# yhwu/rsicnv

Hardware: AMD Instinct MI355X
Metric: bases/sec through RSI pipeline (bin+GC+NB+segment) (higher is better)
Workload: dtype int32

## Files before the change

rsicnv_amd/csrc/kernels.h:

```cpp
#pragma once
#include <hip/hip_runtime.h>
#include <stdint.h>
#include <mutex>
#include "device_util.h"
#include "bam_walk_core.h"

namespace rsik {

inline void note_launch() {
  const hipError_t e = hipGetLastError();
  if (e != hipSuccess && tl_launch_error == hipSuccess) tl_launch_error = e;
}
inline void drain_stale_errors() { (void)hipGetLastError(); tl_launch_error = hipSuccess; }
inline hipError_t take_launch_error() { const hipError_t e = tl_launch_error; tl_launch_error = hipSuccess; return e; }
#define RSI_LAUNCH(...) do { hipLaunchKernelGGL(__VA_ARGS__); rsik::note_launch(); } while (0)

constexpr int kGcLevels = 202;
constexpr int kHistValues = 65536;
constexpr int kResClasses = 32;
constexpr int kTileBases = 4096;

void launch_fasta_classify(const uint8_t* fasta, int64_t n, uint64_t* gcbits, uint64_t* nbits, int64_t nwords,
                           const FillList& fill, hipStream_t stream);
void launch_fill(const FillList& fill, hipStream_t stream);
// ... 149 lines not shown
                    double dup_raw, double RDmedian, void* ws, uint32_t* rawmin_bits, const GridChain& c, GridMedian* g,
                    const GridExport* ex, const FillList* fill, hipStream_t stream);
void launch_nb_apply(const int64_t* binsum, int64_t nb, int64_t K, const void* ws, float* T, const FillList* fill, hipStream_t stream);

struct ScanParams {
  int64_t nb;
  int32_t Lmax;
  int16_t pad;
  int16_t kcap;
  double tmedian;
  double lim_del;
  double lim_dup;
};
constexpr int kMaxScanL = 10400;
constexpr int kScanLdsL = 3800;
constexpr int kScanPad = 8;
constexpr int kThrInline = 232;
struct ScanThr { double del[kThrInline]; double dup[kThrInline]; };
void launch_rsi_scan(const float* T, const int32_t* medint, const ScanParams& sp, const double* thr_del,
                     const double* thr_dup, const ScanThr* inl, uint32_t* first_del, uint32_t* first_dup, uint32_t* counters,
                     uint32_t* tiles, void* tile_ws , hipStream_t stream);
size_t scan_tile_workspace_bytes(int Lmax);
constexpr int kMaxLevels = 10416;
inline int scan_level_stride(int Lmax) { return (Lmax + 1 + kScanPad + 3) & ~3; }
constexpr int kScanRecEscapes = 0, kScanRecInexact = 1, kScanRecStop = 2 , kScanRecTiles = 8, kScanRecLevels = 16;
constexpr size_t kScanWorkBytes = 64 + 2 * (size_t)kMaxLevels * 4;
void launch_level_stop(const uint32_t* first_del, const uint32_t* first_dup, int64_t nb, int32_t Lmax, uint32_t* work, void* both,
                       unsigned int* counter, void* host_copy, size_t host_bytes, hipStream_t stream);
void launch_resolve_runs(const uint32_t* first_del, const uint32_t* first_dup, const uint32_t* levels, int64_t nb, int32_t* status,
                         int32_t* copy, uint64_t* runs, uint32_t* count, uint32_t cap, unsigned int* counter, void* host_copy,
                         uint32_t host_entries, hipStream_t stream);

struct BestSeg { double score; int32_t start; int32_t len; };
struct SegItem { int32_t run; int32_t len; int32_t Lbeg; int32_t Lend; };
constexpr int kRunsInline = 200, kItemsInline = 150;
constexpr int kBestLds = 6144;
struct RunsInline { int32_t se[2 * kRunsInline]; int32_t off[kRunsInline]; };
struct ItemsInline { SegItem it[kItemsInline]; int32_t off[kRunsInline]; };
void launch_run_prefix(const float* T, const int32_t* run_start, const int32_t* run_end, const RunsInline* inl, int nruns,
                       const int64_t* poff, double* scratch, const int32_t* status, int32_t* status_out, hipStream_t stream);
void launch_best_items(const void* items, const ItemsInline* inl, int nitems, const int64_t* poff, const double* scratch,
                       double tmedian, BestSeg* out, hipStream_t stream);
void launch_trim_runs(const float* T, int32_t* status, const int32_t* run_start, const int32_t* run_end, const RunsInline* inl,
                      int nruns, double delthr, double addthr, hipStream_t stream);

size_t level_sums_head_bytes(int Lmax_cap);
size_t level_sums_workspace_bytes(int64_t nb, int32_t clist_cap, int Lmax_cap);
void launch_level_sums(const float* T, const int32_t* status, int64_t nb, int Lmax, void* ws, int Lmax_cap, int32_t clist_cap, float* out,
                       unsigned int* counter, void* host_copy, hipStream_t stream);

constexpr int kMaxDevices = 16;
void report_attribute_failure(const char* kernel, const char* what);
#define RSI_ALLOW_FULL_LDS(kernel)                                                                                  \
  do {                                                                                                              \
    static std::once_flag once__[rsik::kMaxDevices];                                                                \
    int dev__ = 0;                                                                                                  \
    if (hipGetDevice(&dev__) != hipSuccess || dev__ < 0 || dev__ >= rsik::kMaxDevices) dev__ = 0;                   \
    std::call_once(once__[dev__], [dev__] {                                                                         \
      hipFuncAttributes a__;                                                                                        \
      int lds__ = 0;                                                                                                \
      if (hipFuncGetAttributes(&a__, reinterpret_cast<const void*>(kernel)) != hipSuccess) {                        \
        rsik::report_attribute_failure(#kernel, "hipFuncGetAttributes"); return;                                    \
      }                                                                                                             \
      if (hipDeviceGetAttribute(&lds__, hipDeviceAttributeMaxSharedMemoryPerBlock, dev__) != hipSuccess || lds__ <= 0) \
        lds__ = 160 * 1024;                                                                                         \
      if (hipFuncSetAttribute(reinterpret_cast<const void*>(kernel), hipFuncAttributeMaxDynamicSharedMemorySize,   \
                              lds__ - (int)a__.sharedSizeBytes) != hipSuccess)                                      \
        rsik::report_attribute_failure(#kernel, "hipFuncSetAttribute(MaxDynamicSharedMemorySize)");                 \
    });                                                                                                             \
  } while (0)

constexpr unsigned kCandHistBins = 16384;
struct EdgeJob {
  int32_t start, end, type, pad;
};
struct CandJob {
  int32_t start, end;
  int32_t kind;
  int32_t margin;
  int32_t capacity;
  int32_t top;
  int32_t nleft, nright;
  int32_t left_off, right_off;
  int32_t budget;
  int32_t cut;
  double right_cap;
  int64_t iscratch_off;
  int64_t lscratch_off;
};
struct CandOut {
  int32_t flags;
  int32_t nref, nbody, nwin, left_reach, right_reach, body_min, body_max;
  double body_q[3], body_s1, body_s2;
  double ref_q[3], ref_s1, ref_s2;
};
struct DepthRef { const void* p; int bytes; };
void launch_widen_u8(const uint8_t* src, int64_t n, int32_t* dst, hipStream_t stream);
void launch_patch_i32(int32_t* dst, const int32_t* pos, const int32_t* val, int64_t cnt, hipStream_t stream);
void launch_range_sums(DepthRef rdc, const void* ranges , int nranges, long long* sums, hipStream_t stream);
void launch_sharpen_edges(DepthRef rdc, int64_t ncompact, EdgeJob* jobs, int njobs, void* ws, int ws_jobs, hipStream_t stream);
size_t sharpen_workspace_bytes(int njobs);
size_t sharpen_workspace_zero_bytes(int njobs);
inline size_t cand_scratch_bytes(int top, int capacity, int budget, int value_bytes, bool split) {
  auto up16 = [](size_t x) { return (x + 15) & ~size_t(15); };
  const size_t vb = (size_t)value_bytes;
  return up16((size_t)(top + 1 > 0 ? top + 1 : 0) * vb) + up16((size_t)capacity * 4) +
         up16((size_t)(capacity < budget ? capacity : budget) * vb) + (split ? up16((size_t)capacity * vb) : 0);
}
constexpr int kCandChunks = 16;
struct CandMid {
  int32_t lcnt, lreach, lused, rcnt_max, rreach, rused;
  uint32_t done, body_flags;
  float flo[kCandChunks], fhi[kCandChunks];
  double m1[kCandChunks], m2[kCandChunks];
  int32_t body_min, body_max;
  double body_q[3], body_s1, body_s2;
};
void launch_candidate_test_split(DepthRef rdc, int64_t ncompact, const CandJob* jobs, int njobs, const void* chains,
                                 int32_t* iscratch, double RDmedian, CandMid* mid, uint32_t* ghist,
                                 CandOut* outs, int value_bytes, hipStream_t stream);
void launch_candidate_test(DepthRef rdc, int64_t ncompact, const CandJob* jobs, int njobs, const void* chains,
                           int32_t* iscratch, long long* lscratch, double RDmedian, CandOut* outs, int value_bytes, hipStream_t stream);

struct TextParseStats { unsigned long long lines, stored, beyond; unsigned int unsorted, pad; };
int text_parse_workgroups(long long nbytes);
void launch_parse_depth_text(const void* text, long long nbytes, long long size, int32_t* depth, long long* wg_first,
                             long long* wg_max, TextParseStats* stats, hipStream_t stream);

struct NameBound { long long line; int32_t name, len; };
void launch_text_name_bounds(const void* text, long long nbytes, NameBound* bounds, unsigned int* count, unsigned int cap,
                             hipStream_t stream, bool bedgraph = false);
struct GenomeSeg { long long start, n; int32_t* depth; int32_t slot, pad; };
struct GenomeSlotStats { unsigned long long lines, stored, beyond; unsigned int unsorted, pad; long long last_pos;  };
constexpr int kMaxGenomeSegs = 512;
constexpr int kMaxGenomeSamples = 64;
// ... 162 lines not shown
```

rsicnv_amd/csrc/kernels_bin.hip:

```cpp
#include <type_traits>
#include "kernels.h"
#include "device_util.h"

namespace rsik {

namespace {

constexpr int kThreads = 256;
constexpr int kMaxGrid = 256 * 2;

__device__ inline int lane_id() { return threadIdx.x & 63; }
inline int grid_for(int64_t items, int per_block) {
  int64_t g = (items + per_block - 1) / per_block;
  if (g < 1) g = 1;
  if (g > kMaxGrid) g = kMaxGrid;
  return (int)g;
}

__device__ inline uint32_t f32_key(float f) {
  const uint32_t b = __float_as_uint(f);
  return (b & 0x80000000u) ? ~b : (b | 0x80000000u);
}

__device__ __forceinline__ float nb_raw_value(double sum, double m2, double r) {
// ... 1176 lines not shown
                                                        const int32_t* __restrict__ run_end, int nruns, double delthr,
                                                        double addthr, RunsInline inl) {
  __shared__ int s_min[kThreads / 64];
  const int r = blockIdx.x;
  if (r >= nruns) return;
  const int s = run_start ? run_start[r] : inl.se[2 * r], e = run_start ? run_end[r] : inl.se[2 * r + 1];
  auto pred = [&](int i) { const int st = status[i]; const double t = (double)T[i]; return (t > delthr && st < 0) || (t < addthr && st > 0); };
  auto first_failure = [&](int origin, int dir, int limit) {
    int done = 0;
    while (done < limit) {
      const int i = done + (int)threadIdx.x;
      int f = (i < limit && pred(origin + dir * i)) ? 0x7fffffff : i;
      for (int d = 32; d >= 1; d >>= 1) { const int o = __shfl_xor(f, d); f = o < f ? o : f; }
      __syncthreads();
      if ((threadIdx.x & 63) == 0) s_min[threadIdx.x >> 6] = f;
      __syncthreads();
      f = s_min[0];
      for (int w = 1; w < kThreads / 64; ++w) f = s_min[w] < f ? s_min[w] : f;
      if (f != 0x7fffffff) return f < limit ? f : limit;
      done += kThreads;
    }
    return limit;
  };
  const int lim_left = s < e ? e - s : 1;
  const int zl = first_failure(s, +1, lim_left);
  const int L = s + zl;
  int zr = 0;
  if (s < e) zr = first_failure(e, -1, e - L > 1 ? e - L : 1);
  __syncthreads();
  for (int i = threadIdx.x; i < zl; i += kThreads) status[s + i] = 0;
  for (int i = threadIdx.x; i < zr; i += kThreads) status[e - i] = 0;
}

__global__ __launch_bounds__(kThreads) void k_run_prefix(const float* __restrict__ T, const int32_t* __restrict__ run_start,
                                                         const int32_t* __restrict__ run_end,
                                                         const int64_t* __restrict__ poff, double* __restrict__ scratch, RunsInline inl,
                                                         const int32_t* __restrict__ status, int32_t* __restrict__ status_out) {
  __shared__ double s_tot[kThreads];
  const int r = blockIdx.x;
  const int s = run_start ? run_start[r] : inl.se[2 * r];
  const int len = (run_start ? run_end[r] : inl.se[2 * r + 1]) - s + 1;
  const int64_t off = poff ? poff[r] : (int64_t)inl.off[r];
  double* P = scratch + off;
  if (status_out) for (int e = threadIdx.x; e < len; e += kThreads) status_out[off - r + e] = status[s + e];
  const int chunk = (len + kThreads - 1) / kThreads;
  const int c0 = threadIdx.x * chunk;
  double run = 0.0;
  for (int e = c0; e < c0 + chunk && e < len; ++e) run += (double)T[s + e];
  s_tot[threadIdx.x] = run;
  __syncthreads();
  if (threadIdx.x < 64) {
    double carry = 0.0;
    for (int k = 0; k < kThreads / 64; ++k) {
      const double mine = s_tot[k * 64 + threadIdx.x];
      const double incl = wave_incl_scan(mine);
      s_tot[k * 64 + threadIdx.x] = carry + incl - mine;
      carry += wave_lane63(incl);
    }
  }
  __syncthreads();
  run = s_tot[threadIdx.x];
  if (threadIdx.x == 0) P[0] = 0.0;
  for (int e = c0; e < c0 + chunk && e < len; ++e) { run += (double)T[s + e]; P[e + 1] = run; }
}

__device__ inline bool seg_better(double s, int L, int j, double bs, int bL, int bj) {
  if (s != bs) return s > bs;
  if (L != bL) return L < bL;
  return j < bj;
}

__global__ __launch_bounds__(kThreads) void k_best_subsegment(const SegItem* __restrict__ items,
                                                              const int64_t* __restrict__ poff,
                                                              const double* __restrict__ scratch, double tmedian,
                                                              BestSeg* __restrict__ out, ItemsInline inl) {
  __shared__ double s_s[kThreads];
  __shared__ int s_L[kThreads], s_j[kThreads];
  const SegItem it = items ? items[blockIdx.x] : inl.it[blockIdx.x];
  const double* P = scratch + (poff ? poff[it.run] : (int64_t)inl.off[it.run]);
  double bs = -1.0; int bL = 0x7fffffff, bj = 0x7fffffff;
  __shared__ double s_P[kBestLds];
  const bool staged = it.len + 1 <= kBestLds;
  if (staged) for (int e = threadIdx.x; e <= it.len; e += kThreads) s_P[e] = P[e];
  __syncthreads();
  const double* Q = staged ? s_P : P;
  for (int L0 = it.Lbeg; L0 < it.Lend; L0 += 4) {
    double dL[4], sq[4];
#pragma unroll
    for (int u = 0; u < 4; ++u) { dL[u] = (double)(L0 + u); sq[u] = sqrt(dL[u]); }
    for (int j = threadIdx.x; j + L0 <= it.len; j += kThreads) {
      const double pj = Q[j];
      double sum[4];
#pragma unroll
      for (int u = 0; u < 4; ++u) { const int L = L0 + u; sum[u] = (L < it.Lend && j + L <= it.len) ? Q[j + L] - pj : 0.0; }
#pragma unroll
      for (int u = 0; u < 4; ++u) {
        const int L = L0 + u;
        if (L < it.Lend && j + L <= it.len) {
          const double score = fabs(sum[u] / dL[u] - tmedian) * sq[u];
          if (seg_better(score, L, j, bs, bL, bj)) { bs = score; bL = L; bj = j; }
        }
      }
    }
  }
  s_s[threadIdx.x] = bs; s_L[threadIdx.x] = bL; s_j[threadIdx.x] = bj;
  __syncthreads();
  for (int d = kThreads / 2; d >= 1; d >>= 1) {
    if ((int)threadIdx.x < d) {
      if (seg_better(s_s[threadIdx.x + d], s_L[threadIdx.x + d], s_j[threadIdx.x + d], s_s[threadIdx.x], s_L[threadIdx.x], s_j[threadIdx.x])) {
        s_s[threadIdx.x] = s_s[threadIdx.x + d]; s_L[threadIdx.x] = s_L[threadIdx.x + d]; s_j[threadIdx.x] = s_j[threadIdx.x + d];
      }
    }
    __syncthreads();
  }
  if (threadIdx.x == 0) { out[blockIdx.x].score = s_s[0]; out[blockIdx.x].start = s_j[0]; out[blockIdx.x].len = s_L[0]; }
}
// ... 150 lines not shown
               counters, list, parts, inl ? *inl : none, gws, gbytes); } while (0)
  if (gtile && sh.wide) RSI_SCAN(false, true, true, thr_del, thr_dup);
  else if (gtile) { if (inl) RSI_SCAN(true, true, false, nullptr, nullptr); else RSI_SCAN(false, true, false, thr_del, thr_dup); }
  else { if (inl) RSI_SCAN(true, false, false, nullptr, nullptr); else RSI_SCAN(false, false, false, thr_del, thr_dup); }
#undef RSI_SCAN
}
void launch_level_stop(const uint32_t* first_del, const uint32_t* first_dup, int64_t nb, int32_t Lmax, uint32_t* work, void* both,
                       unsigned int* counter, void* host_copy, size_t host_bytes, hipStream_t stream) {
  const size_t lds = (size_t)(Lmax + 1) * 8;
  if (lds + 256 <= 160 * 1024) {
    RSI_ALLOW_FULL_LDS(k_level_stop<false>);
    RSI_LAUNCH(k_level_stop<false>, dim3(grid_for(nb, kThreads * 16)), dim3(kThreads), lds, stream, first_del, first_dup, nb,
                       Lmax, work, static_cast<uint2*>(both), counter, host_copy, (unsigned int)host_bytes);
  } else {
    RSI_LAUNCH(k_level_stop<true>, dim3(grid_for(nb, kThreads * 16)), dim3(kThreads), 0, stream, first_del, first_dup, nb,
                       Lmax, work, static_cast<uint2*>(both), counter, host_copy, (unsigned int)host_bytes);
  }
}
void launch_resolve_runs(const uint32_t* first_del, const uint32_t* first_dup, const uint32_t* levels, int64_t nb, int32_t* status,
                         int32_t* copy, uint64_t* runs, uint32_t* count, uint32_t cap, unsigned int* counter, void* host_copy,
                         uint32_t host_entries, hipStream_t stream) {
  RSI_LAUNCH(k_resolve_runs, dim3(grid_for(nb, kThreads * 4)), dim3(kThreads), 0, stream, first_del, first_dup, levels, nb, status, copy,
                     runs, count, cap, counter, host_copy, host_entries);
}
void launch_trim_runs(const float* T, int32_t* status, const int32_t* run_start, const int32_t* run_end, const RunsInline* inl, int nruns,
                      double delthr, double addthr, hipStream_t stream) {
  if (nruns <= 0) return;
  static const RunsInline none{};
  RSI_LAUNCH(k_trim_runs, dim3(nruns), dim3(kThreads), 0, stream, T, status, run_start, run_end,
                     nruns, delthr, addthr, inl ? *inl : none);
}

void launch_run_prefix(const float* T, const int32_t* run_start, const int32_t* run_end, const RunsInline* inl, int nruns, const int64_t* poff,
                       double* scratch, const int32_t* status, int32_t* status_out, hipStream_t stream) {
  if (nruns <= 0) return;
  static const RunsInline none{};
  RSI_LAUNCH(k_run_prefix, dim3(nruns), dim3(kThreads), 0, stream, T, run_start, run_end, poff, scratch, inl ? *inl : none, status, status_out);
}
void launch_best_items(const void* items, const ItemsInline* inl, int nitems, const int64_t* poff, const double* scratch, double tmedian,
                       BestSeg* out, hipStream_t stream) {
  if (nitems <= 0) return;
  static const ItemsInline none{};
  RSI_LAUNCH(k_best_subsegment, dim3(nitems), dim3(kThreads), 0, stream, reinterpret_cast<const SegItem*>(items), poff,
                     scratch, tmedian, out, inl ? *inl : none);
}

}
```

rsicnv_amd/csrc/kernels_cand.hip:

```cpp
#include "kernels.h"

namespace rsik {

namespace {

constexpr int kThreads = 256;
constexpr int kTestThreads = 1024;
constexpr int kMaxWaves = kTestThreads / 64;
__device__ inline int lane_id() { return threadIdx.x & 63; }

template <class T, class Op>
__device__ inline T block_reduce(T v, Op op, T* s_tmp ) {
  for (int d = 32; d >= 1; d >>= 1) v = op(v, __shfl_xor(v, d));
  __syncthreads();
  if (lane_id() == 0) s_tmp[threadIdx.x >> 6] = v;
  __syncthreads();
  T r = s_tmp[0];
  for (int w = 1; w < (int)(blockDim.x >> 6); ++w) r = op(r, s_tmp[w]);
  __syncthreads();
  return r;
}
__device__ inline int block_exscan(int v, int* s_tmp , int* total) {
  const int incl = wave_incl_scan(v);
  __syncthreads();
// ... 661 lines not shown
template <typename TS> struct CandRun16;
template <> struct CandRun16<uint8_t> {
  uint32_t w[4];
  __device__ inline void clear() { w[0] = w[1] = w[2] = w[3] = 0u; }
  __device__ inline void load(const uint8_t* p) { const WalkBytes16 b = *reinterpret_cast<const WalkBytes16*>(p); w[0] = b.w[0]; w[1] = b.w[1]; w[2] = b.w[2]; w[3] = b.w[3]; }
  __device__ inline void put(int k, int x) { w[k >> 2] |= (uint32_t)x << (8 * (k & 3)); }
  __device__ inline int get(int k) const { return (int)((w[k >> 2] >> (8 * (k & 3))) & 0xffu); }
  __device__ inline long long sum() const {
    unsigned s = 0;
#pragma unroll
    for (int q = 0; q < 4; ++q) s = __builtin_amdgcn_sad_u8(w[q], 0u, s);
    return (long long)s;
  }
};
template <> struct CandRun16<int32_t> {
  int v[16];
  __device__ inline void clear() {
#pragma unroll
    for (int k = 0; k < 16; ++k) v[k] = 0;
  }
  __device__ inline void load(const int32_t* p) {
#pragma unroll
    for (int q = 0; q < 4; ++q) { const WalkInts4 b = *reinterpret_cast<const WalkInts4*>(p + 4 * q); v[4 * q] = b.x; v[4 * q + 1] = b.y; v[4 * q + 2] = b.z; v[4 * q + 3] = b.w; }
  }
  __device__ inline void put(int k, int x) { v[k] = x; }
  __device__ inline int get(int k) const { return v[k]; }
  __device__ inline long long sum() const {
    long long s = 0;
#pragma unroll
    for (int k = 0; k < 16; ++k) s += v[k];
    return s;
  }
};
template <typename TS>
__device__ inline void cand_load16(const CandJob& J, const CandGeom& g, const TS* __restrict__ left, const TS* __restrict__ right,
                                   int i0, int lim, CandRun16<TS>& r) {
  if (!g.thin && i0 + 16 <= lim && (i0 + 16 <= g.used0 || i0 >= g.used0)) {
    r.load(i0 < g.used0 ? left + (J.top + 1 - g.used0 + i0) : right + (i0 - g.used0));
  } else {
    r.clear();
#pragma unroll
    for (int k = 0; k < 16; ++k) if (i0 + k < lim) r.put(k, cand_value(J, g, left, right, i0 + k));
  }
}

__device__ inline int cand_sum_chunks(const CandGeom& g) {
  const long long fit = 4ll * g.nref / g.width;
  return fit < kCandChunks ? (int)fit : kCandChunks;
}
__device__ inline int cand_sum_chunk_len(int nwin, int chunks) { return (((nwin + chunks - 1) / chunks) + 3) & ~3; }

template <typename TD, typename TS>
__global__ __launch_bounds__(kTestThreads) void k_cand_sums(const TD* __restrict__ A, const CandJob* __restrict__ jobs,
                                                        int32_t* __restrict__ iscratch, CandMid* __restrict__ mid) {
  extern __shared__ unsigned int s_hist[];
  __shared__ long long s_l[kMaxWaves];
  __shared__ int s_i2[kMaxWaves];
  __shared__ int s_scan[kMaxWaves];
  __shared__ int s_q[3];
  const CandJob J = jobs[blockIdx.y];
  CandMid& M = mid[blockIdx.y];
  const CandGeom g = cand_geometry(J, M);
  const CandBufs b = cand_buffers(J, iscratch, nullptr, (int)sizeof(TS));
  const TS* const left = reinterpret_cast<const TS*>(b.left);
  const TS* const right = reinterpret_cast<const TS*>(b.right);
  if (g.nwin <= 0 || g.width <= 0) return;
// ... 230 lines not shown
  for (unsigned e = threadIdx.x; e < nbk; e += kTestThreads) ghist[e] = 0;
  if (threadIdx.x == 0) { M.done = 0; outs[blockIdx.y] = O; }
}

template <typename TD>
__global__ __launch_bounds__(kThreads) void k_range_sums(const TD* __restrict__ A, const int2* __restrict__ ranges,
                                                         long long* __restrict__ sums) {
  __shared__ long long s_l[kThreads / 64 + 1];
  const int2 r = ranges[blockIdx.x];
  long long acc = 0;
  for (int p = r.x + (int)threadIdx.x; p <= r.y; p += kThreads) acc += A[p];
  acc = block_reduce(acc, [](long long a, long long b) { return a + b; }, s_l);
  if (threadIdx.x == 0) sums[blockIdx.x] = acc;
}

}

#define RSI_DEPTH_DISPATCH(D, CALL32, CALL8) do { if ((D).bytes == 1) { const uint8_t* rdc = static_cast<const uint8_t*>((D).p); CALL8; } \
                                                 else { const int32_t* rdc = static_cast<const int32_t*>((D).p); CALL32; } } while (0)

void launch_range_sums(DepthRef d, const void* ranges, int nranges, long long* sums, hipStream_t stream) {
  if (nranges <= 0) return;
  RSI_DEPTH_DISPATCH(d,
    RSI_LAUNCH(k_range_sums<int32_t>, dim3(nranges), dim3(kThreads), 0, stream, rdc, static_cast<const int2*>(ranges), sums),
    RSI_LAUNCH(k_range_sums<uint8_t>, dim3(nranges), dim3(kThreads), 0, stream, rdc, static_cast<const int2*>(ranges), sums));
}

void launch_sharpen_edges(DepthRef d, int64_t ncompact, EdgeJob* jobs, int njobs, void* ws, int ws_jobs, hipStream_t stream) {
  if (njobs <= 0) return;
  RSI_DEPTH_DISPATCH(d,
    RSI_LAUNCH(k_sharpen_edges<int32_t>, dim3(2 * kEdgeChunks, njobs), dim3(kThreads), 0, stream, rdc, ncompact, jobs, ws_jobs, ws),
    RSI_LAUNCH(k_sharpen_edges<uint8_t>, dim3(2 * kEdgeChunks, njobs), dim3(kThreads), 0, stream, rdc, ncompact, jobs, ws_jobs, ws));
}
namespace {
template <typename TD, typename TS>
void cand_launch_split(const TD* rdc, int64_t ncompact, const CandJob* jobs, int njobs, const int2* ch, int32_t* iscratch,
                       double RDmedian, CandMid* mid, uint32_t* ghist, CandOut* outs, hipStream_t stream) {
  const size_t lds = (size_t)kCandHistBins * 4;
  RSI_ALLOW_FULL_LDS((k_cand_gather<TD, TS>));
  RSI_ALLOW_FULL_LDS((k_cand_sums<TD, TS>));
  RSI_ALLOW_FULL_LDS(k_cand_hist);
  const int vb = (int)sizeof(TS);
  long long* const lscratch = nullptr;
  RSI_LAUNCH((k_cand_gather<TD, TS>), dim3(2, njobs), dim3(kTestThreads), lds, stream, rdc, ncompact, jobs, ch, iscratch, lscratch, RDmedian, mid);
  RSI_LAUNCH((k_cand_sums<TD, TS>), dim3(kCandChunks + 1, njobs), dim3(kTestThreads), lds, stream, rdc, jobs, iscratch, mid);
  RSI_LAUNCH(k_cand_hist, dim3(kCandChunks, njobs), dim3(kTestThreads), lds, stream, jobs, iscratch, lscratch, mid, ghist, outs, vb);
}
template <typename TD, typename TS>
void cand_launch_one_wg(const TD* rdc, int64_t ncompact, const CandJob* jobs, int njobs, const int2* ch, int32_t* iscratch,
                        long long* lscratch, double RDmedian, CandOut* outs, hipStream_t stream) {
  const size_t lds = (size_t)kCandHistBins * 4;
  RSI_ALLOW_FULL_LDS((k_candidate_test<TD, TS>));
  RSI_LAUNCH((k_candidate_test<TD, TS>), dim3(njobs), dim3(kTestThreads), lds, stream, rdc, ncompact, jobs, ch, iscratch, lscratch, RDmedian, outs);
}
}
void launch_candidate_test_split(DepthRef d, int64_t ncompact, const CandJob* jobs, int njobs, const void* chains,
                                 int32_t* iscratch, double RDmedian, CandMid* mid, uint32_t* ghist,
                                 CandOut* outs, int value_bytes, hipStream_t stream) {
  if (njobs <= 0) return;
  const int2* ch = static_cast<const int2*>(chains);
  if (d.bytes == 1 && value_bytes == 1)
    cand_launch_split<uint8_t, uint8_t>(static_cast<const uint8_t*>(d.p), ncompact, jobs, njobs, ch, iscratch, RDmedian, mid, ghist, outs, stream);
  else if (d.bytes == 1)
    cand_launch_split<uint8_t, int32_t>(static_cast<const uint8_t*>(d.p), ncompact, jobs, njobs, ch, iscratch, RDmedian, mid, ghist, outs, stream);
  else
    cand_launch_split<int32_t, int32_t>(static_cast<const int32_t*>(d.p), ncompact, jobs, njobs, ch, iscratch, RDmedian, mid, ghist, outs, stream);
// ... 45 lines not shown
```

rsicnv_amd/csrc/pipeline.hip:

```cpp
#include <new>
#include "pipeline_internal.h"
#include "geno_host.h"
#include "pipeline_steps.h"

using namespace rsik;
using namespace rsip;
using rsih::Candidate;
using rsih::Region;

namespace {

struct ScanOut {
  double tmedian1 = 0, tsigma1 = 0, tlamda1 = 0, tmedian2 = 0, tsigma2 = 0, tlamda2 = 0;
  int Lmax = 0;
  rsih::IntSpan status2;
  std::vector<int> run_status;
  std::vector<rsih::IntSpan::Range> run_ranges;
  std::vector<Candidate> segs;
  uint32_t escapes = 0, inexact = 0;
  uint32_t tiles_listed = 0;
  std::vector<uint32_t> level_log[4];
  uint32_t stop_levels[4] = {0, 0, 0, 0};
  std::vector<std::string> fs_lines;
};
// ... 196 lines not shown

constexpr size_t kCandScratchBytes = size_t(512) << 20;
class DeviceTester : public rsih::NeighbourTester {
 public:
  DeviceTester(rsi_ctx* c, DepthRef rdc, int64_t n, double RDmedian) : ctx(c), d_rdc(rdc), N(n), median(RDmedian) {}
  double kernel_wait_ms = 0;
  int launches = 0;
  int force_split = -1, force_bytes = -1;
  std::vector<CandOut>* sink = nullptr;
  int mailbox_lists = 0, copied_lists = 0;

  bool sharpen(std::vector<Candidate>& L) override {
    if (L.empty()) return true;
    const int nj = (int)L.size();
    EdgeJob* slot = static_cast<EdgeJob*>(mb_alloc(ctx, (size_t)nj * sizeof(EdgeJob)));
    std::vector<EdgeJob> spill;
    EdgeJob* jobs = slot;
    if (!slot) { spill.resize((size_t)nj); jobs = spill.data(); }
    for (int i = 0; i < nj; ++i) jobs[i] = {L[(size_t)i].start, L[(size_t)i].end, L[(size_t)i].type, 0};
    {
      Phase ph(ctx, "cand.ensure");
      if (nj > ctx->sharpen_ws_jobs) {
        const int cap = std::max(256, 2 * nj);
        if (!ok(ctx->sharpen_ws.ensure(sharpen_workspace_bytes(cap)))) return false;
        if (!ok(hipMemsetAsync(ctx->sharpen_ws.p, 0, sharpen_workspace_zero_bytes(cap), ctx->stream))) return false;
        ctx->sharpen_ws_jobs = cap;
      }
      if (!slot && !ok(ctx->cand_jobs.ensure((size_t)nj * sizeof(EdgeJob)))) return false;
    }
    GateShared gs(ctx);
    Phase ph(ctx, "cand.sharpen");
    EdgeJob* d_jobs = slot ? slot : ctx->cand_jobs.as<EdgeJob>();
    if (!slot && !ok(copy_h2d(ctx, ctx->cand_jobs.p, jobs, (size_t)nj * sizeof(EdgeJob)))) return false;
    for (int pass = 0; pass < 2; ++pass) {
      Timer t(ctx, "sharpen_edges");
      launch_sharpen_edges(d_rdc, N, d_jobs, nj, ctx->sharpen_ws.p, ctx->sharpen_ws_jobs, ctx->stream);
    }
    if (!slot && !ok(copy_d2h(ctx, jobs, ctx->cand_jobs.p, (size_t)nj * sizeof(EdgeJob)))) return false;
    if (!wait()) return false;
    gs.release();
    for (int i = 0; i < nj; ++i) { L[(size_t)i].start = jobs[i].start; L[(size_t)i].end = jobs[i].end; }
    return true;
  }

  bool test(const std::vector<rsih::TestPlan>& plans, std::vector<rsih::TestStats>& stats, std::vector<int>& left_reach,
            std::vector<char>& okv) override {
    const size_t n = plans.size();
    stats.assign(n, rsih::TestStats{});
    left_reach.assign(n, 0);
    okv.assign(n, 0);
    const bool split = force_split >= 0 ? force_split != 0 : env_int("RSI_HOT_CAND_SPLIT", 1) != 0;
    if (sink) { CandOut none{}; none.flags = -1; sink->assign(n, none); }
    const int value_bytes = d_rdc.bytes == 1 && (force_bytes >= 0 ? force_bytes != 0 : env_int("RSI_HOT_CAND_BYTES", 1) != 0) ? 1 : 4;
    size_t first = 0;
    while (first < n) {
      std::vector<CandJob> jobs;
      std::vector<int32_t> chains;
      size_t ibytes = 0, lwords = 0, last = first;
      for (; last < n; ++last) {
        const rsih::TestPlan& T = plans[last];
        if (T.capacity <= 0 || T.end < T.start || T.start < 0 || T.end >= N) break;
        auto up4 = [](size_t x) { return (x + 3) & ~(size_t)3; };
        const size_t ib = cand_scratch_bytes(T.top, T.capacity, T.budget, value_bytes, split);
        const size_t lw = split ? 0 : up4((size_t)T.capacity + 1);
        if (!jobs.empty() && ibytes + ib + (lwords + lw) * 8 > kCandScratchBytes) break;
        CandJob J{};
        J.start = T.start; J.end = T.end; J.kind = T.kind; J.margin = T.margin; J.capacity = T.capacity; J.top = T.top;
        J.nleft = (int)T.left_chain.size(); J.nright = (int)T.right_chain.size();
        J.left_off = (int)(chains.size() / 2);
// ... 162 lines not shown
  const size_t work_bytes = 64 + ((size_t)scan_level_stride(Lmax) + (size_t)Lmax + 1) * 4;
  if (scan_tile_workspace_bytes(Lmax)) HIPCHK(ctx->scan_ws.ensure(scan_tile_workspace_bytes(Lmax)));
  uint32_t* rslot = static_cast<uint32_t*>(mb_alloc(ctx, 8 + (size_t)kEagerBounds * 8));
  uint32_t* wslot = static_cast<uint32_t*>(work_bytes <= kMailboxBytes / 8 ? mb_alloc(ctx, work_bytes) : nullptr);
  const bool spilled = !wslot && Lmax > kMaxL && spill;
  if (spilled) spill->assign((work_bytes + 3) / 4, 0u);
  if ((!wslot && !spilled) || !rslot) return fail(ctx, RSI_ERR_INTERNAL, "out of pinned mailbox memory");
  ScanParams sp;
  sp.nb = nb; sp.Lmax = Lmax; sp.pad = 0; sp.tmedian = tmedian;
  sp.lim_del = RDmedian * 0.75; sp.lim_dup = RDmedian * 1.25;
  { Timer t(ctx, "rsi_scan"); launch_rsi_scan(d_T, d_medint, sp, d_del, d_dup, use_inl ? &inl : nullptr, d_first_del, d_first_dup, work, ctx->scan_tiles.as<uint32_t>(), ctx->scan_ws.p, ctx->stream); }
  { Timer t(ctx, "level_stop"); launch_level_stop(d_first_del, d_first_dup, nb, Lmax, work, ctx->runs.p, d_done + 2, wslot, wslot ? work_bytes : 0, ctx->stream); }
  if (spilled) { HIPCHK(hipMemcpyAsync(spill->data(), work, work_bytes, hipMemcpyDeviceToHost, ctx->stream)); wslot = spill->data(); }
  { Timer t(ctx, "resolve_runs"); launch_resolve_runs(d_first_del, d_first_dup, work + 2, nb, d_status, d_copy, ctx->runs.as<uint64_t>(), d_count, kMaxRunEntries, d_done + 3, rslot, kEagerBounds, ctx->stream); }
  *work_slot = wslot; *runs_slot = rslot;
  return RSI_OK;
}

struct SegForm { int runs = 0, items = 0, inl = 0, mailbox_status = 0, unstaged = 0; int64_t pairs_per_item = 0; };
int rsi_segments(rsi_ctx* ctx, const float* d_T, const int32_t* d_st2, int64_t nb, const std::vector<Region>& runs, double tmedian,
                 double tlamda, int64_t pairs_per_item, ScanOut& out, SegForm* form) {
  int rc;
  out.status2 = rsih::IntSpan();
  out.segs.clear();
  if (runs.empty()) return RSI_OK;
  std::vector<int64_t> poff;
  std::vector<SegItem> items;
  if (pairs_per_item <= 0) pairs_per_item = rsih::segment_pairs_per_item(runs, !ctx->gate || ctx->gate->lonely());
  rsih::segment_items(runs, pairs_per_item, poff, items);
  HIPCHK(ctx->scratch.ensure((size_t)poff.back() * 8 + (runs.size() + 1) * 8));
  double* d_scratch = ctx->scratch.as<double>();
  const bool inl = runs.size() <= (size_t)kRunsInline && items.size() <= (size_t)kItemsInline && poff.back() < (int64_t)1 << 31;
  std::vector<BestSeg> best(items.size());
  if (inl) {
    RunArgs ra;
    if ((rc = prepare_runs(ctx, runs, ra)) != RSI_OK) return rc;
    ItemsInline ii;
    memset(&ii, 0, sizeof(ii));
    for (size_t r = 0; r < runs.size(); ++r) { ra.inl.off[r] = (int32_t)poff[r]; ii.off[r] = (int32_t)poff[r]; }
    for (size_t i = 0; i < items.size(); ++i) ii.it[i] = items[i];
    BestSeg* slot = static_cast<BestSeg*>(mb_alloc(ctx, items.size() * sizeof(BestSeg)));
    if (!slot) return fail(ctx, RSI_ERR_INTERNAL, "out of pinned mailbox memory");
    const size_t run_bins = (size_t)(poff.back() - (int64_t)runs.size());
    int32_t* sslot = run_bins * 4 <= kMailboxMaxCopy ? static_cast<int32_t*>(mb_alloc(ctx, std::max<size_t>(run_bins, 1) * 4)) : nullptr;
    if (!sslot) {
      HIPCHK(ctx->h_status2.ensure((size_t)nb * 4));
      HIPCHK(hipMemcpyAsync(ctx->h_status2.p, d_st2, (size_t)nb * 4, hipMemcpyDeviceToHost, ctx->stream));
    }
    { Timer t(ctx, "run_prefix"); launch_run_prefix(d_T, nullptr, nullptr, &ra.inl, (int)runs.size(), nullptr, d_scratch, d_st2, sslot, ctx->stream); }
    { Timer t(ctx, "best_subsegment"); launch_best_items(nullptr, &ii, (int)items.size(), nullptr, d_scratch, tmedian, slot, ctx->stream); }
    HIPCHK(CTX_SYNC());
    memcpy(best.data(), slot, items.size() * sizeof(BestSeg));
    if (sslot) {
      out.run_status.assign(sslot, sslot + run_bins);
      out.run_ranges.clear();
      for (size_t r = 0; r < runs.size(); ++r) out.run_ranges.push_back({runs[r].start, runs[r].end, poff[r] - (int64_t)r});
      out.status2 = rsih::IntSpan(out.run_status.data(), nb, &out.run_ranges);
    } else {
      out.status2 = rsih::IntSpan(ctx->h_status2.as<int>(), nb);
    }
  } else {
    RunArgs ra;
    const size_t kr = runs.size();
    HIPCHK(ctx->run_se.ensure(kr * 8 + 64));
    std::vector<int32_t> se(2 * kr);
    for (size_t i = 0; i < kr; ++i) { se[i] = runs[i].start; se[kr + i] = runs[i].end; }
    HIPCHK(copy_h2d(ctx, ctx->run_se.p, se.data(), kr * 8));
    int64_t* d_poff = reinterpret_cast<int64_t*>(d_scratch + poff.back());
    HIPCHK(ctx->items.ensure(items.size() * sizeof(SegItem)));
    HIPCHK(ctx->best.ensure(items.size() * sizeof(BestSeg)));
    HIPCHK(copy_h2d(ctx, d_poff, poff.data(), poff.size() * 8));
    HIPCHK(copy_h2d(ctx, ctx->items.p, items.data(), items.size() * sizeof(SegItem)));
    HIPCHK(ctx->h_status2.ensure((size_t)nb * 4));
    HIPCHK(hipMemcpyAsync(ctx->h_status2.p, d_st2, (size_t)nb * 4, hipMemcpyDeviceToHost, ctx->stream));
    out.status2 = rsih::IntSpan(ctx->h_status2.as<int>(), nb);
    { Timer t(ctx, "run_prefix"); launch_run_prefix(d_T, ctx->run_se.as<int32_t>(), ctx->run_se.as<int32_t>() + kr, nullptr, (int)kr, d_poff, d_scratch, nullptr, nullptr, ctx->stream); }
    { Timer t(ctx, "best_subsegment"); launch_best_items(ctx->items.p, nullptr, (int)items.size(), d_poff, d_scratch, tmedian, ctx->best.as<BestSeg>(), ctx->stream); }
    HIPCHK(copy_d2h(ctx, best.data(), ctx->best.p, items.size() * sizeof(BestSeg)));
    HIPCHK(CTX_SYNC());
  }
  if (form) {
    form->runs = (int)runs.size(); form->items = (int)items.size(); form->inl = inl ? 1 : 0;
    form->mailbox_status = out.status2.ranges ? 1 : 0;
    form->pairs_per_item = pairs_per_item;
    for (const Region& r : runs) if (r.end - r.start + 2 > kBestLds) ++form->unstaged;
  }
  rsih::segments_from_best(runs, items, best.data(), out.status2, tlamda, out.segs);
  return RSI_OK;
}

struct FsForm { int runs = -1, inl = -1, copied = -1, route = 0, has_level0 = 0, trim = 0, leveldel = 0, leveladd = 0; float m0 = 0.0f; };
template <class Synced>
int rsi_filterstatus(rsi_ctx* ctx, const float* d_T, const int32_t* d_st1, int32_t* d_st1f, int64_t nb, int Lmax, double dev,
                     const uint32_t* rslot, Synced&& synced, std::vector<std::string>* fs_lines, FsForm* form) {
  int rc;
  const bool long_scan = Lmax > kMaxL;
  const int nlev = 2 * Lmax + 1;
  uint32_t* fs_slot = long_scan ? nullptr : static_cast<uint32_t*>(mb_alloc(ctx, (size_t)nlev * 8));
  if (!fs_slot && !long_scan) return fail(ctx, RSI_ERR_INTERNAL, "out of pinned mailbox memory");
  if (!long_scan) {
    GateShared gs(ctx);
    Timer t(ctx, "level_sums");
    launch_level_sums(d_T, d_st1, nb, Lmax, ctx->fs_ws.p, kMaxL, kFsListCap, ctx->fs_out.as<float>(),
                      reinterpret_cast<unsigned int*>(ctx->small.as<uint8_t>() + kOffDone) + kDoneBinSlot + 4, fs_slot, ctx->stream);
  }
  { Phase phc(ctx, "fs.wait"); HIPCHK(CTX_SYNC()); }
  if ((rc = synced()) != RSI_OK) return rc;
  {
    Phase phs(ctx, "fs.sums");
    std::vector<float> wsum((size_t)nlev, 0.0f);
    std::vector<int> wcnt((size_t)nlev, 0);
    if (fs_slot) {
      memcpy(wsum.data(), fs_slot, (size_t)nlev * 4);
      memcpy(wcnt.data(), fs_slot + nlev, (size_t)nlev * 4);
    }
    if (form) form->route = long_scan ? 2 : (wcnt[(size_t)Lmax] < 0 ? 1 : 0);
    if (long_scan || wcnt[(size_t)Lmax] < 0) {
      Phase phc(ctx, "fs.copy");
// ... 1956 lines not shown
```

rsicnv_amd/csrc/pipeline_steps.h:

```cpp
#pragma once
#include <math.h>
#include <stdio.h>
#include <string.h>
#include <algorithm>
#include <string>
#include <vector>
#include "host_calls.h"
#include "hostmath.h"
#include "kernels.h"

namespace rsih {

inline bool boundary_pairs(const uint64_t* raw, size_t cnt, bool end_exclusive, std::vector<Region>& out) {
  out.clear();
  std::vector<int64_t> s, e;
  for (size_t i = 0; i < cnt; ++i) { const uint64_t v = raw[i]; ((v & 1) ? e : s).push_back((int64_t)(v >> 1)); }
  if (s.size() != e.size()) return false;
  std::sort(s.begin(), s.end());
  std::sort(e.begin(), e.end());
  for (size_t i = 0; i < s.size(); ++i) out.push_back({(int)s[i], (int)(e[i] - (end_exclusive ? 1 : 0))});
  return true;
}

inline float unkey_f32(uint32_t k) {
// ... 198 lines not shown
  int leveldel = lo, leveladd = hi;
  for (int l = 0; l < nl; ++l) if (lsum[l] < m0 - dev) { leveldel = l + lo; break; }
  for (int l = nl - 1; l >= 0; --l) if (lsum[l] > m0 + dev) { leveladd = l + lo; break; }
  char line[128];
  for (int l = 0; l < nl; ++l) if (lcnt[l] != 0) { snprintf(line, sizeof(line), "%d\t%d\t%g", l + lo, lcnt[l], (double)lsum[l]); c.lines.push_back(line); }
  snprintf(line, sizeof(line), "%d\t%g", leveldel, (double)lsum[leveldel - lo]); c.lines.push_back(line);
  snprintf(line, sizeof(line), "%d\t%g", leveladd, (double)lsum[leveladd - lo]); c.lines.push_back(line);
  c.trim = !(leveldel > 0 || leveladd < 0 || leveldel > leveladd);
  if (!c.trim) c.lines.push_back("warning level error, status not filtered");
  c.m0 = m0; c.leveldel = leveldel; c.leveladd = leveladd;
  return c;
}

inline int64_t segment_pairs_per_item(const std::vector<Region>& runs, bool lonely) {
  int64_t pairs_per_item = 1 << 16;
  if (lonely) {
    int64_t total = 0;
    for (const Region& r : runs) { const int64_t len = r.end - r.start + 1; total += len * (len + 1) / 2; }
    const int64_t room = std::max<int64_t>(8, (int64_t)rsik::kItemsInline - 2 * (int64_t)runs.size());
    pairs_per_item = std::min<int64_t>(pairs_per_item, std::max<int64_t>(1 << 13, total / room + 1));
  }
  return pairs_per_item;
}
inline void segment_items(const std::vector<Region>& runs, int64_t pairs_per_item, std::vector<int64_t>& poff, std::vector<rsik::SegItem>& items) {
  poff.assign(runs.size() + 1, 0);
  items.clear();
  for (size_t r = 0; r < runs.size(); ++r) {
    const int len = runs[r].end - runs[r].start + 1;
    poff[r + 1] = poff[r] + len + 1;
    int L = 1;
    while (L <= len) {
      int64_t pairs = 0; int Le = L;
      while (Le <= len && pairs < pairs_per_item) { pairs += len - Le + 1; ++Le; }
      items.push_back({(int32_t)r, (int32_t)len, (int32_t)L, (int32_t)Le});
      L = Le;
    }
  }
}
inline void segments_from_best(const std::vector<Region>& runs, const std::vector<rsik::SegItem>& items, const rsik::BestSeg* best,
                               const IntSpan& status2, double tlamda, std::vector<Candidate>& segs) {
  std::vector<rsik::BestSeg> per_run(runs.size(), rsik::BestSeg{-1.0, 0, 0});
  for (size_t i = 0; i < items.size(); ++i) {
    rsik::BestSeg& b = per_run[(size_t)items[i].run];
    if (best[i].score > b.score) b = best[i];
  }
  for (size_t r = 0; r < runs.size(); ++r) {
    Candidate c;
    const int len = runs[r].end - runs[r].start + 1;
    double sc = per_run[r].score;
    if (sc > 0) { c.start = runs[r].start + per_run[r].start; c.end = c.start + per_run[r].len - 1; }
    else { c.start = runs[r].start; c.end = runs[r].start + len - 1; sc = 0; }
    const Quantiles q = grid_quantiles(status2.at(c.start), (size_t)(c.end - c.start + 1));
    if (q.med > 0) { c.type = kDup; c.score = sc; } else { c.type = kDel; c.score = -sc; }
    if (fabs(c.score) < tlamda * 0.5) continue;
    segs.push_back(c);
  }
}

}
```

Before: 282.7 billion.

## Fold run prefix sums into best-subsegment kernel and add single-launch edge sharpening

The segmentation step now computes each run's prefix sums directly in LDS inside the best-subsegment kernel, and exports status there too. The separate run_prefix launch is kept only for runs too long to stage in LDS. A separate change adds a one-block-per-job edge sharpening kernel that does both passes in one launch when all jobs are short enough, replacing two multi-block sharpen_edges launches. The cost is that items sharing a run each recompute its prefix, and the inline kernel-argument struct grows.

```diff
diff --git a/rsicnv_amd/csrc/kernels.h b/rsicnv_amd/csrc/kernels.h
--- a/rsicnv_amd/csrc/kernels.h
+++ b/rsicnv_amd/csrc/kernels.h
@@ -205,15 +205,17 @@
                          uint32_t host_entries, hipStream_t stream);
 
 struct BestSeg { double score; int32_t start; int32_t len; };
-struct SegItem { int32_t run; int32_t len; int32_t Lbeg; int32_t Lend; };
+struct SegItem { int32_t run; int32_t len; int32_t Lbeg; int32_t Lend; int32_t start; };
 constexpr int kRunsInline = 200, kItemsInline = 150;
 constexpr int kBestLds = 6144;
 struct RunsInline { int32_t se[2 * kRunsInline]; int32_t off[kRunsInline]; };
 struct ItemsInline { SegItem it[kItemsInline]; int32_t off[kRunsInline]; };
+static_assert(sizeof(ItemsInline) + 8 * 8 <= 4096, "k_best_subsegment's arguments must stay under the 4 KB kernel-argument limit");
 void launch_run_prefix(const float* T, const int32_t* run_start, const int32_t* run_end, const RunsInline* inl, int nruns,
-                       const int64_t* poff, double* scratch, const int32_t* status, int32_t* status_out, hipStream_t stream);
+                       const int64_t* poff, double* scratch, const int32_t* status, int32_t* status_out, int unstaged_only,
+                       hipStream_t stream);
 void launch_best_items(const void* items, const ItemsInline* inl, int nitems, const int64_t* poff, const double* scratch,
-                       double tmedian, BestSeg* out, hipStream_t stream);
+                       double tmedian, BestSeg* out, const float* T, const int32_t* status, int32_t* status_out, hipStream_t stream);
 void launch_trim_runs(const float* T, int32_t* status, const int32_t* run_start, const int32_t* run_end, const RunsInline* inl,
                       int nruns, double delthr, double addthr, hipStream_t stream);
 
@@ -274,6 +276,9 @@
 void launch_sharpen_edges(DepthRef rdc, int64_t ncompact, EdgeJob* jobs, int njobs, void* ws, int ws_jobs, hipStream_t stream);
 size_t sharpen_workspace_bytes(int njobs);
 size_t sharpen_workspace_zero_bytes(int njobs);
+constexpr int kSharpenOneMaxLen = 1 << 15;
+constexpr int kSharpenOneMaxLenInt32 = 1 << 14;
+void launch_sharpen_one(DepthRef rdc, int64_t ncompact, EdgeJob* jobs, int njobs, hipStream_t stream);
 inline size_t cand_scratch_bytes(int top, int capacity, int budget, int value_bytes, bool split) {
   auto up16 = [](size_t x) { return (x + 15) & ~size_t(15); };
   const size_t vb = (size_t)value_bytes;
diff --git a/rsicnv_amd/csrc/kernels_bin.hip b/rsicnv_amd/csrc/kernels_bin.hip
--- a/rsicnv_amd/csrc/kernels_bin.hip
+++ b/rsicnv_amd/csrc/kernels_bin.hip
@@ -1232,17 +1232,7 @@
   for (int i = threadIdx.x; i < zr; i += kThreads) status[e - i] = 0;
 }
 
-__global__ __launch_bounds__(kThreads) void k_run_prefix(const float* __restrict__ T, const int32_t* __restrict__ run_start,
-                                                         const int32_t* __restrict__ run_end,
-                                                         const int64_t* __restrict__ poff, double* __restrict__ scratch, RunsInline inl,
-                                                         const int32_t* __restrict__ status, int32_t* __restrict__ status_out) {
-  __shared__ double s_tot[kThreads];
-  const int r = blockIdx.x;
-  const int s = run_start ? run_start[r] : inl.se[2 * r];
-  const int len = (run_start ? run_end[r] : inl.se[2 * r + 1]) - s + 1;
-  const int64_t off = poff ? poff[r] : (int64_t)inl.off[r];
-  double* P = scratch + off;
-  if (status_out) for (int e = threadIdx.x; e < len; e += kThreads) status_out[off - r + e] = status[s + e];
+__device__ inline void run_prefix_block(const float* __restrict__ T, int s, int len, double* P, double* s_tot) {
   const int chunk = (len + kThreads - 1) / kThreads;
   const int c0 = threadIdx.x * chunk;
   double run = 0.0;
@@ -1263,6 +1253,23 @@
   if (threadIdx.x == 0) P[0] = 0.0;
   for (int e = c0; e < c0 + chunk && e < len; ++e) { run += (double)T[s + e]; P[e + 1] = run; }
 }
+__device__ inline void run_status_export(const int32_t* __restrict__ status, int32_t* __restrict__ status_out, int s, int len, int64_t off, int r) {
+  for (int e = threadIdx.x; e < len; e += kThreads) status_out[off - r + e] = status[s + e];
+}
+
+__global__ __launch_bounds__(kThreads) void k_run_prefix(const float* __restrict__ T, const int32_t* __restrict__ run_start,
+                                                         const int32_t* __restrict__ run_end,
+                                                         const int64_t* __restrict__ poff, double* __restrict__ scratch, RunsInline inl,
+                                                         const int32_t* __restrict__ status, int32_t* __restrict__ status_out, int unstaged_only) {
+  __shared__ double s_tot[kThreads];
+  const int r = blockIdx.x;
+  const int s = run_start ? run_start[r] : inl.se[2 * r];
+  const int len = (run_start ? run_end[r] : inl.se[2 * r + 1]) - s + 1;
+  const int64_t off = poff ? poff[r] : (int64_t)inl.off[r];
+  if (status_out) run_status_export(status, status_out, s, len, off, r);
+  if (unstaged_only && len + 1 <= kBestLds) return;
+  run_prefix_block(T, s, len, scratch + off, s_tot);
+}
 
 __device__ inline bool seg_better(double s, int L, int j, double bs, int bL, int bj) {
   if (s != bs) return s > bs;
@@ -1273,15 +1280,22 @@
 __global__ __launch_bounds__(kThreads) void k_best_subsegment(const SegItem* __restrict__ items,
                                                               const int64_t* __restrict__ poff,
                                                               const double* __restrict__ scratch, double tmedian,
-                                                              BestSeg* __restrict__ out, ItemsInline inl) {
+                                                              BestSeg* __restrict__ out, ItemsInline inl,
+                                                              const float* __restrict__ T, const int32_t* __restrict__ status,
+                                                              int32_t* __restrict__ status_out) {
   __shared__ double s_s[kThreads];
   __shared__ int s_L[kThreads], s_j[kThreads];
   const SegItem it = items ? items[blockIdx.x] : inl.it[blockIdx.x];
-  const double* P = scratch + (poff ? poff[it.run] : (int64_t)inl.off[it.run]);
+  const int64_t off = poff ? poff[it.run] : (int64_t)inl.off[it.run];
+  const double* P = scratch + off;
   double bs = -1.0; int bL = 0x7fffffff, bj = 0x7fffffff;
   __shared__ double s_P[kBestLds];
   const bool staged = it.len + 1 <= kBestLds;
-  if (staged) for (int e = threadIdx.x; e <= it.len; e += kThreads) s_P[e] = P[e];
+  if (T && status_out && it.Lbeg == 1) run_status_export(status, status_out, it.start, it.len, off, it.run);
+  if (staged) {
+    if (T) run_prefix_block(T, it.start, it.len, s_P, s_s);
+    else for (int e = threadIdx.x; e <= it.len; e += kThreads) s_P[e] = P[e];
+  }
   __syncthreads();
   const double* Q = staged ? s_P : P;
   for (int L0 = it.Lbeg; L0 < it.Lend; L0 += 4) {
@@ -1498,17 +1512,18 @@
 }
 
 void launch_run_prefix(const float* T, const int32_t* run_start, const int32_t* run_end, const RunsInline* inl, int nruns, const int64_t* poff,
-                       double* scratch, const int32_t* status, int32_t* status_out, hipStream_t stream) {
+                       double* scratch, const int32_t* status, int32_t* status_out, int unstaged_only, hipStream_t stream) {
   if (nruns <= 0) return;
   static const RunsInline none{};
-  RSI_LAUNCH(k_run_prefix, dim3(nruns), dim3(kThreads), 0, stream, T, run_start, run_end, poff, scratch, inl ? *inl : none, status, status_out);
+  RSI_LAUNCH(k_run_prefix, dim3(nruns), dim3(kThreads), 0, stream, T, run_start, run_end, poff, scratch, inl ? *inl : none, status, status_out,
+                     unstaged_only);
 }
 void launch_best_items(const void* items, const ItemsInline* inl, int nitems, const int64_t* poff, const double* scratch, double tmedian,
-                       BestSeg* out, hipStream_t stream) {
+                       BestSeg* out, const float* T, const int32_t* status, int32_t* status_out, hipStream_t stream) {
   if (nitems <= 0) return;
   static const ItemsInline none{};
   RSI_LAUNCH(k_best_subsegment, dim3(nitems), dim3(kThreads), 0, stream, reinterpret_cast<const SegItem*>(items), poff,
-                     scratch, tmedian, out, inl ? *inl : none);
-}
-
-}
+                     scratch, tmedian, out, inl ? *inl : none, T, status, status_out);
+}
+
+}
diff --git a/rsicnv_amd/csrc/kernels_cand.hip b/rsicnv_amd/csrc/kernels_cand.hip
--- a/rsicnv_amd/csrc/kernels_cand.hip
+++ b/rsicnv_amd/csrc/kernels_cand.hip
@@ -717,6 +717,90 @@
     return s;
   }
 };
+constexpr int kSharpenOneThreads = 512;
+template <typename TD>
+__device__ inline int sharpen_window(const TD* __restrict__ rdc, int64_t N, int from, int len, int wbase, int wend, bool want_max,
+                                     long long* s_l, long long* s_v, int* s_i) {
+  const int T = (int)blockDim.x, tid = (int)threadIdx.x;
+  auto inside = [&](long long first) { return first >= 0 && first + 15 <= (long long)N - 1; };
+  auto at = [&](long long pos) { return (long long)rdc[pos < 0 ? 0 : (pos > (long long)N - 1 ? (long long)N - 1 : pos)]; };
+  long long acc = 0;
+  {
+    const long long q0 = (long long)from + wbase;
+    for (int j0 = tid * 16; j0 < len; j0 += T * 16) {
+      if (j0 + 16 <= len && inside(q0 - len + j0) && inside(q0 + j0)) {
+        CandRun16<TD> left, right;
+        left.load(rdc + (q0 - len + j0));
+        right.load(rdc + (q0 + j0));
+        acc += left.sum() - right.sum();
+      } else {
+        for (int j = j0; j < j0 + 16 && j < len; ++j) acc += at(q0 - len + j) - at(q0 + j);
+      }
+    }
+  }
+  const long long dd0 = block_reduce(acc, [](long long a, long long b) { return a + b; }, s_l);
+  const int wspan = wend > wbase ? wend - wbase : 0;
+  const int share = (((wspan + T - 1) / T) + 15) & ~15;
+  const int a = wbase + tid * share;
+  ArgBest best{0, -1};
+  long long cur = 0;
+  for (int k = 0; k < share && a + k < wend; k += 16) {
+    const int i0 = a + k;
+    const long long q = (long long)from + i0;
+    if (i0 + 16 <= wend && inside(q - len) && inside(q) && inside(q + len)) {
+      CandRun16<TD> lo, mid, hi;
+      lo.load(rdc + (q - len));
+      mid.load(rdc + q);
+      hi.load(rdc + (q + len));
+#pragma unroll
+      for (int j = 0; j < 16; ++j) {
+        if (best.i < 0 || (want_max ? cur > best.v : cur < best.v)) { best.v = cur; best.i = i0 + j; }
+        cur += -(long long)lo.get(j) + 2ll * mid.get(j) - (long long)hi.get(j);
+      }
+    } else {
+      for (int i = i0; i < i0 + 16 && i < wend; ++i) {
+        if (best.i < 0 || (want_max ? cur > best.v : cur < best.v)) { best.v = cur; best.i = i; }
+        const long long p = (long long)from + i;
+        cur += -at(p - len) + 2ll * at(p) - at(p + len);
+      }
+    }
+  }
+  long long total;
+  const long long ex = block_exscan_i64(cur, s_l, &total);
+  best.v += dd0 + ex;
+  if (best.i >= 0 && !(want_max ? best.v > 0 : best.v < 0)) best.i = -1;
+  for (int d = 32; d >= 1; d >>= 1) { ArgBest o; o.v = __shfl_xor(best.v, d); o.i = __shfl_xor(best.i, d); best = arg_pick(best, o, want_max); }
+  if (lane_id() == 0) { s_v[tid >> 6] = best.v; s_i[tid >> 6] = best.i; }
+  __syncthreads();
+  ArgBest r{s_v[0], s_i[0]};
+  for (int w = 1; w < (T >> 6); ++w) r = arg_pick(r, ArgBest{s_v[w], s_i[w]}, want_max);
+  __syncthreads();
+  return r.i;
+}
+
+template <typename TD>
+__global__ __launch_bounds__(kSharpenOneThreads) void k_sharpen_one(const TD* __restrict__ rdc, int64_t ncompact, EdgeJob* __restrict__ jobs) {
+  __shared__ long long s_l[kMaxWaves];
+  __shared__ long long s_v[kMaxWaves];
+  __shared__ int s_i[kMaxWaves];
+  const EdgeJob job = jobs[blockIdx.x];
+  if (job.type > 1) return;
+  const bool del = job.type == 0;
+  int start = job.start, end = job.end;
+  for (int call = 0; call < 2; ++call) {
+    const int len = end - start + 1;
+    const int reach = len / 4 > 250 ? len / 4 : 250;
+    const int from = start - reach, to = end + reach;
+    if (from < 2 * len || (int64_t)to > ncompact - 2 * (int64_t)len) break;
+    const int nstep = to - from, wlen = 2 * reach;
+    const int pick0 = sharpen_window(rdc, ncompact, from, len, 0, wlen < nstep ? wlen : nstep, del, s_l, s_v, s_i);
+    const int pick1 = sharpen_window(rdc, ncompact, from, len, nstep - wlen > 0 ? nstep - wlen : 0, nstep, !del, s_l, s_v, s_i);
+    if (pick0 > 0) start = from + pick0;
+    if (pick1 > 0) end = to - nstep + pick1;
+  }
+  if (threadIdx.x == 0) { jobs[blockIdx.x].start = start; jobs[blockIdx.x].end = end; }
+}
+
 template <typename TS>
 __device__ inline void cand_load16(const CandJob& J, const CandGeom& g, const TS* __restrict__ left, const TS* __restrict__ right,
                                    int i0, int lim, CandRun16<TS>& r) {
@@ -1013,6 +1097,12 @@
     RSI_LAUNCH(k_sharpen_edges<int32_t>, dim3(2 * kEdgeChunks, njobs), dim3(kThreads), 0, stream, rdc, ncompact, jobs, ws_jobs, ws),
     RSI_LAUNCH(k_sharpen_edges<uint8_t>, dim3(2 * kEdgeChunks, njobs), dim3(kThreads), 0, stream, rdc, ncompact, jobs, ws_jobs, ws));
 }
+void launch_sharpen_one(DepthRef d, int64_t ncompact, EdgeJob* jobs, int njobs, hipStream_t stream) {
+  if (njobs <= 0) return;
+  RSI_DEPTH_DISPATCH(d,
+    RSI_LAUNCH(k_sharpen_one<int32_t>, dim3(njobs), dim3(kSharpenOneThreads), 0, stream, rdc, ncompact, jobs),
+    RSI_LAUNCH(k_sharpen_one<uint8_t>, dim3(njobs), dim3(kSharpenOneThreads), 0, stream, rdc, ncompact, jobs));
+}
 namespace {
 template <typename TD, typename TS>
 void cand_launch_split(const TD* rdc, int64_t ncompact, const CandJob* jobs, int njobs, const int2* ch, int32_t* iscratch,
diff --git a/rsicnv_amd/csrc/pipeline.hip b/rsicnv_amd/csrc/pipeline.hip
--- a/rsicnv_amd/csrc/pipeline.hip
+++ b/rsicnv_amd/csrc/pipeline.hip
@@ -252,9 +252,16 @@
     Phase ph(ctx, "cand.sharpen");
     EdgeJob* d_jobs = slot ? slot : ctx->cand_jobs.as<EdgeJob>();
     if (!slot && !ok(copy_h2d(ctx, ctx->cand_jobs.p, jobs, (size_t)nj * sizeof(EdgeJob)))) return false;
-    for (int pass = 0; pass < 2; ++pass) {
-      Timer t(ctx, "sharpen_edges");
-      launch_sharpen_edges(d_rdc, N, d_jobs, nj, ctx->sharpen_ws.p, ctx->sharpen_ws_jobs, ctx->stream);
+    int64_t longest = 0;
+    for (int i = 0; i < nj; ++i) longest = std::max<int64_t>(longest, (int64_t)jobs[i].end - jobs[i].start + 1);
+    if (!env_off("RSI_HOT_SHARPEN_ONE") && longest <= (int64_t)env_int("RSI_HOT_SHARPEN_ONE_MAX", d_rdc.bytes == 1 ? kSharpenOneMaxLen : kSharpenOneMaxLenInt32)) {
+      Timer t(ctx, "sharpen_one");
+      launch_sharpen_one(d_rdc, N, d_jobs, nj, ctx->stream);
+    } else {
+      for (int pass = 0; pass < 2; ++pass) {
+        Timer t(ctx, "sharpen_edges");
+        launch_sharpen_edges(d_rdc, N, d_jobs, nj, ctx->sharpen_ws.p, ctx->sharpen_ws_jobs, ctx->stream);
+      }
     }
     if (!slot && !ok(copy_d2h(ctx, jobs, ctx->cand_jobs.p, (size_t)nj * sizeof(EdgeJob)))) return false;
     if (!wait()) return false;
@@ -483,6 +490,9 @@
   double* d_scratch = ctx->scratch.as<double>();
   const bool inl = runs.size() <= (size_t)kRunsInline && items.size() <= (size_t)kItemsInline && poff.back() < (int64_t)1 << 31;
   std::vector<BestSeg> best(items.size());
+  const bool fold = !env_off("RSI_HOT_SEG_FOLD");
+  int unstaged = 0;
+  for (const Region& r : runs) if (r.end - r.start + 2 > kBestLds) ++unstaged;
   if (inl) {
     RunArgs ra;
     if ((rc = prepare_runs(ctx, runs, ra)) != RSI_OK) return rc;
@@ -498,8 +508,9 @@
       HIPCHK(ctx->h_status2.ensure((size_t)nb * 4));
       HIPCHK(hipMemcpyAsync(ctx->h_status2.p, d_st2, (size_t)nb * 4, hipMemcpyDeviceToHost, ctx->stream));
     }
-    { Timer t(ctx, "run_prefix"); launch_run_prefix(d_T, nullptr, nullptr, &ra.inl, (int)runs.size(), nullptr, d_scratch, d_st2, sslot, ctx->stream); }
-    { Timer t(ctx, "best_subsegment"); launch_best_items(nullptr, &ii, (int)items.size(), nullptr, d_scratch, tmedian, slot, ctx->stream); }
+    if (!fold) { Timer t(ctx, "run_prefix"); launch_run_prefix(d_T, nullptr, nullptr, &ra.inl, (int)runs.size(), nullptr, d_scratch, d_st2, sslot, 0, ctx->stream); }
+    else if (unstaged) { Timer t(ctx, "run_prefix"); launch_run_prefix(d_T, nullptr, nullptr, &ra.inl, (int)runs.size(), nullptr, d_scratch, nullptr, nullptr, 1, ctx->stream); }
+    { Timer t(ctx, "best_subsegment"); launch_best_items(nullptr, &ii, (int)items.size(), nullptr, d_scratch, tmedian, slot, fold ? d_T : nullptr, d_st2, sslot, ctx->stream); }
     HIPCHK(CTX_SYNC());
     memcpy(best.data(), slot, items.size() * sizeof(BestSeg));
     if (sslot) {
@@ -525,8 +536,8 @@
     HIPCHK(ctx->h_status2.ensure((size_t)nb * 4));
     HIPCHK(hipMemcpyAsync(ctx->h_status2.p, d_st2, (size_t)nb * 4, hipMemcpyDeviceToHost, ctx->stream));
     out.status2 = rsih::IntSpan(ctx->h_status2.as<int>(), nb);
-    { Timer t(ctx, "run_prefix"); launch_run_prefix(d_T, ctx->run_se.as<int32_t>(), ctx->run_se.as<int32_t>() + kr, nullptr, (int)kr, d_poff, d_scratch, nullptr, nullptr, ctx->stream); }
-    { Timer t(ctx, "best_subsegment"); launch_best_items(ctx->items.p, nullptr, (int)items.size(), d_poff, d_scratch, tmedian, ctx->best.as<BestSeg>(), ctx->stream); }
+    if (!fold || unstaged) { Timer t(ctx, "run_prefix"); launch_run_prefix(d_T, ctx->run_se.as<int32_t>(), ctx->run_se.as<int32_t>() + kr, nullptr, (int)kr, d_poff, d_scratch, nullptr, nullptr, fold ? 1 : 0, ctx->stream); }
+    { Timer t(ctx, "best_subsegment"); launch_best_items(ctx->items.p, nullptr, (int)items.size(), d_poff, d_scratch, tmedian, ctx->best.as<BestSeg>(), fold ? d_T : nullptr, nullptr, nullptr, ctx->stream); }
     HIPCHK(copy_d2h(ctx, best.data(), ctx->best.p, items.size() * sizeof(BestSeg)));
     HIPCHK(CTX_SYNC());
   }
@@ -534,7 +545,7 @@
     form->runs = (int)runs.size(); form->items = (int)items.size(); form->inl = inl ? 1 : 0;
     form->mailbox_status = out.status2.ranges ? 1 : 0;
     form->pairs_per_item = pairs_per_item;
-    for (const Region& r : runs) if (r.end - r.start + 2 > kBestLds) ++form->unstaged;
+    form->unstaged = unstaged;
   }
   rsih::segments_from_best(runs, items, best.data(), out.status2, tlamda, out.segs);
   return RSI_OK;
diff --git a/rsicnv_amd/csrc/pipeline_steps.h b/rsicnv_amd/csrc/pipeline_steps.h
--- a/rsicnv_amd/csrc/pipeline_steps.h
+++ b/rsicnv_amd/csrc/pipeline_steps.h
@@ -254,7 +254,7 @@
     while (L <= len) {
       int64_t pairs = 0; int Le = L;
       while (Le <= len && pairs < pairs_per_item) { pairs += len - Le + 1; ++Le; }
-      items.push_back({(int32_t)r, (int32_t)len, (int32_t)L, (int32_t)Le});
+      items.push_back({(int32_t)r, (int32_t)len, (int32_t)L, (int32_t)Le, (int32_t)runs[r].start});
       L = Le;
     }
   }
```

Result: no change. 284.0 billion (median of 6 runs) (+0.5%).
